# SonyCSLParis/audio-metrics

Measured on AMD Instinct MI355X. Metric: evaluate() embeddings/sec (FAD+KD+PRDC), 2×100k CLAP-512 sets, 1/2/4/8 GPUs, higher is better.
Workload: dtype f32

## Files before the change

audio-metrics_amd/csrc/am_common.h:

```cpp
#pragma once
#include <hip/hip_runtime.h>
#include <stdint.h>
#include <stddef.h>
#include <stdio.h>
#include "../../include/audio_metrics_hip.h"

namespace am {

char* last_error_buf();
void set_error(const char* fmt, ...);

#define AM_HIP_TRY(expr)                                                             \
    do {                                                                             \
        hipError_t _e = (expr);                                                      \
        if (_e != hipSuccess) {                                                      \
            am::set_error("%s failed: %s (%s:%d)", #expr, hipGetErrorString(_e),     \
                          __FILE__, __LINE__);                                       \
            return AM_ERR_HIP;                                                       \
        }                                                                            \
    } while (0)

#define AM_LAUNCH_CHECK()                                                            \
    do {                                                                             \
        hipError_t _e = hipGetLastError();                                           \
// ... 1 lines not shown
            am::set_error("kernel launch failed: %s (%s:%d)", hipGetErrorString(_e), \
                          __FILE__, __LINE__);                                       \
            return AM_ERR_HIP;                                                       \
        }                                                                            \
    } while (0)

#define AM_REQUIRE(cond, status, ...)                                                \
    do {                                                                             \
        if (!(cond)) {                                                               \
            am::set_error(__VA_ARGS__);                                              \
            return (status);                                                         \
        }                                                                            \
    } while (0)

hipError_t ensure_dynamic_lds(const void* kernel, int bytes);

void clock_begin(int kernel, hipStream_t st);
void clock_end(int kernel, hipStream_t st);

__device__ __forceinline__ float clamp0(float v) { return v != v ? __builtin_inff() : fmaxf(v, 0.f); }

static inline bool aligned16(const void* p) { return (reinterpret_cast<uintptr_t>(p) & 15u) == 0; }
static inline size_t round_up(size_t x, size_t a) { return (x + a - 1) / a * a; }
static inline int64_t ceil_div(int64_t a, int64_t b) { return (a + b - 1) / b; }

struct Carver {
    char* base;
    size_t size;
    size_t off = 0;
    Carver(void* p, size_t n) : base(static_cast<char*>(p)), size(n) {}
    template <class T>
    T* take(size_t count) {
        size_t bytes = round_up(count * sizeof(T), 256);
        T* r = (base && off + bytes <= size) ? reinterpret_cast<T*>(base + off) : nullptr;
        off += bytes;
        return r;
    }
    bool ok() const { return base != nullptr && off <= size; }
};

bool knn64_filter_eligible(int64_t N, int D, int k);
size_t knn64_filter_workspace(int64_t N, int D, int k);
int knn64_filter(const double* X, int64_t N, int64_t ld, int D, int k, double* out_r, void* ws, size_t ws_bytes, hipStream_t st);
bool prdc64_filter_eligible(int64_t Nr, int64_t Nc, int D);
size_t prdc64_filter_workspace(int64_t Nr, int64_t Nc, int D);
int prdc64_filter(const double* R, int64_t Nr, int64_t ldr, const double* C, int64_t Nc, int64_t ldc, int D, const double* rt,
                  const double* ct, int32_t* col_count, unsigned* row_any, unsigned* row_cover, const int** fail_flag, void* ws,
                  size_t ws_bytes, hipStream_t st);
size_t knn64_self_workspace(int64_t N, int k);
int knn64_self_gated(const double* X, int64_t N, int64_t ld, int D, int k, double* out_r, void* ws, size_t ws_bytes, const int* run_flag,
                     hipStream_t st);


}
```

audio-metrics_amd/csrc/evaluate.hip:

```cpp
#include "am_common.h"
#include <algorithm>
#include <vector>

namespace am {

__global__ void eval_pack_kernel(const double* __restrict__ fad5, const long long* __restrict__ totals, double* __restrict__ out,
                                 unsigned what) {
    const int t = threadIdx.x;
    if (t < AM_EVAL_HEAD) {
        double v = 0.0;
        if (t < 5) v = (what & AM_EVAL_FAD) ? fad5[t] : (t == 4 ? -1.0 : 0.0);
        else if (t < 9) v = (what & AM_EVAL_PRDC) ? (double)totals[t - 5] : 0.0;
        out[t] = v;
    }
}

struct EvalLayout {
    size_t total = 0;
    size_t stats_ws = 0, knn_ws = 0, prdc_ws = 0, kd_ws = 0, fad_ws = 0;
    double *mean[2] = {nullptr, nullptr}, *cov[2] = {nullptr, nullptr};
    float *norms[2] = {nullptr, nullptr}, *radii[2] = {nullptr, nullptr};
    uint32_t* pstats[2] = {nullptr, nullptr};
    uint16_t* half[2] = {nullptr, nullptr};
    int32_t* col = nullptr;
    uint8_t *rany = nullptr, *rcov = nullptr;
    long long* totals = nullptr;
    double* fad_out = nullptr;
    void *ws_main = nullptr, *ws_fad = nullptr;
    size_t ws_main_bytes = 0;
};

static bool eval_layout(Carver& c, int64_t n_ref, int64_t n_cand, int D, int k, int S, int m, unsigned what, EvalLayout& L) {
    const int64_t n[2] = {n_ref, n_cand};
    for (int s = 0; s < 2; ++s) {
        L.mean[s] = c.take<double>(D);
        L.cov[s] = c.take<double>((size_t)D * D);
    }
    size_t main_bytes = 0;
    if (what & AM_EVAL_FAD) {
        main_bytes = std::max({main_bytes, am_stats_workspace_bytes(n_ref, D), am_stats_workspace_bytes(n_cand, D)});
        L.fad_ws = am_frechet_workspace_bytes(D);
        L.ws_fad = c.take<char>(L.fad_ws);
        L.fad_out = c.take<double>(8);
    }
    if (what & AM_EVAL_PRDC) {
        const int64_t ldh = am_prepared_half_ld(D);
        for (int s = 0; s < 2; ++s) {
            L.norms[s] = c.take<float>(n[s]);
            L.pstats[s] = c.take<uint32_t>(4);
            L.half[s] = c.take<uint16_t>((size_t)n[s] * ldh);
            L.radii[s] = c.take<float>(n[s]);
        }
        L.col = c.take<int32_t>(n_cand);
        L.rany = c.take<uint8_t>(n_ref);
        L.rcov = c.take<uint8_t>(n_ref);
        L.totals = c.take<long long>(4);
        main_bytes = std::max({main_bytes, am_knn_workspace_bytes(n_ref, n_ref, D, k), am_knn_workspace_bytes(n_cand, n_cand, D, k),
                               am_prdc_workspace_bytes(n_ref, n_cand, D)});
    }
    if (what & AM_EVAL_KD) main_bytes = std::max(main_bytes, am_kd_poly_workspace_bytes(S, m, D));
    L.ws_main_bytes = round_up(std::max<size_t>(main_bytes, 256), 256);
    L.ws_main = c.take<char>(L.ws_main_bytes);
    L.total = c.off;
    return c.ok();
}

}

using namespace am;

extern "C" size_t am_evaluate_workspace_bytes(int64_t n_ref, int64_t n_cand, int D, int nearest_k, int kd_subsets, int kd_m,
                                              unsigned what) {
    if (n_ref < 1 || n_cand < 1 || D < 1) return 0;
    Carver c(nullptr, 0);
    EvalLayout L;
    eval_layout(c, n_ref, n_cand, D, nearest_k, kd_subsets, kd_m, what, L);
    return L.total;
}

extern "C" int am_evaluate_f32(const float* ref, int64_t n_ref, int64_t ld_ref, const float* cand, int64_t n_cand,
                               int64_t ld_cand, int D, unsigned what, int nearest_k, const int64_t* idx_cand,
                               const int64_t* idx_ref, int kd_subsets, int kd_m, double kd_gamma, double kd_coef0, int kd_degree,
                               const am_evaluate_side* given_ref, const am_evaluate_side* given_cand, double* out, void* ws,
                               size_t ws_bytes, am_stream_t stream, am_stream_t side_stream) {
    AM_REQUIRE(ref && cand && out, AM_ERR_BAD_ARG, "null pointer");
    AM_REQUIRE(n_ref >= 1 && n_cand >= 1 && D >= 1, AM_ERR_BAD_SHAPE, "sets of %lld and %lld rows x %d", (long long)n_ref,
               (long long)n_cand, D);
    AM_REQUIRE((what & ~(unsigned)(AM_EVAL_FAD | AM_EVAL_KD | AM_EVAL_PRDC)) == 0 && what != 0, AM_ERR_BAD_ARG, "what = %u", what);
    AM_REQUIRE(!(what & AM_EVAL_KD) || (idx_cand && idx_ref && kd_subsets >= 1 && kd_m >= 1), AM_ERR_BAD_ARG,
               "kernel distance needs the two index tables");
    AM_REQUIRE(!(what & AM_EVAL_FAD) || side_stream != stream, AM_ERR_BAD_ARG,
               "the Frechet solve runs on side_stream, which must differ from stream");
    hipStream_t st = static_cast<hipStream_t>(stream), side = static_cast<hipStream_t>(side_stream);
#ifdef AM_DEV_KNOBS
    static const int fad_place = getenv("AM_EVAL_FAD_PLACE") ? atoi(getenv("AM_EVAL_FAD_PLACE")) : 0;
#else
    constexpr int fad_place = 0;
#endif
    Carver c(ws, ws_bytes);
    EvalLayout L;
    AM_REQUIRE(eval_layout(c, n_ref, n_cand, D, nearest_k, kd_subsets, kd_m, what, L), AM_ERR_WORKSPACE,
               "workspace too small: need %zu bytes, have %zu", L.total, ws_bytes);
    const float* X[2] = {ref, cand};
    const int64_t n[2] = {n_ref, n_cand}, ld[2] = {ld_ref, ld_cand};
    const am_evaluate_side* given[2] = {given_ref, given_cand};
    int rc;

    const double* mean[2];
    const double* cov[2];
    if (what & AM_EVAL_FAD) {
        for (int s = 0; s < 2; ++s) {
            if (given[s] && given[s]->mean && given[s]->cov) {
                mean[s] = given[s]->mean;
                cov[s] = given[s]->cov;
                continue;
            }
            double* m_out = given[s] && given[s]->mean_out ? given[s]->mean_out : L.mean[s];
            double* c_out = given[s] && given[s]->cov_out ? given[s]->cov_out : L.cov[s];
            if ((rc = am_stats_f32(X[s], n[s], D, ld[s], m_out, c_out, L.ws_main, L.ws_main_bytes, stream)) != AM_OK) return rc;
            mean[s] = m_out;
            cov[s] = c_out;
        }
    }
    struct EventGuard {
        hipEvent_t e = nullptr;
        ~EventGuard() {
            if (e) (void)hipEventDestroy(e);
        }
    } ev_stats, ev_fad;
    if ((what & AM_EVAL_FAD) && fad_place != 2) {
        AM_HIP_TRY(hipEventCreateWithFlags(&ev_stats.e, hipEventDisableTiming));
        AM_HIP_TRY(hipEventRecord(ev_stats.e, st));
    }

    if (what & AM_EVAL_PRDC) {
        am_prepared_set prep[2];
        for (int s = 0; s < 2; ++s) {
            if ((rc = am_prepare_set_f32(X[s], n[s], ld[s], D, L.norms[s], L.pstats[s], L.half[s], stream)) != AM_OK) return rc;
            prep[s].norms = L.norms[s];
            prep[s].stats = L.pstats[s];
            prep[s].half = L.half[s];
        }
        const float* radii[2];
        for (int s = 0; s < 2; ++s) {
            if (given[s] && given[s]->radii) {
                radii[s] = given[s]->radii;
                continue;
            }
            float* r_out = given[s] && given[s]->radii_out ? given[s]->radii_out : L.radii[s];
            if ((rc = am_knn_radii_prepared_f32(X[s], n[s], ld[s], D, &prep[s], nearest_k, r_out, L.ws_main, L.ws_main_bytes,
                                                stream)) != AM_OK)
                return rc;
            radii[s] = r_out;
            if ((what & AM_EVAL_FAD) && fad_place == 2 && ev_stats.e == nullptr) {
                AM_HIP_TRY(hipEventCreateWithFlags(&ev_stats.e, hipEventDisableTiming));
                AM_HIP_TRY(hipEventRecord(ev_stats.e, st));
            }
        }
        if ((rc = am_prdc_counts_prepared_f32(ref, n_ref, ld_ref, &prep[0], cand, n_cand, ld_cand, &prep[1], D, radii[0], radii[1],
                                              L.col, L.rany, L.rcov, nullptr, L.ws_main, L.ws_main_bytes, stream)) != AM_OK)
            return rc;
        if ((rc = am_prdc_reduce(L.col, n_cand, L.rany, L.rcov, n_ref, reinterpret_cast<int64_t*>(L.totals), stream)) != AM_OK)
            return rc;
    }

    if (what & AM_EVAL_KD) {
        if ((rc = am_kd_poly_f32(cand, n_cand, ld_cand, ref, n_ref, ld_ref, D, idx_cand, idx_ref, kd_subsets, kd_m, kd_gamma,
                                 kd_coef0, kd_degree, out + AM_EVAL_HEAD, L.ws_main, L.ws_main_bytes, stream)) != AM_OK)
            return rc;
    }

    if (what & AM_EVAL_FAD) {
        const bool serial = fad_place == 1;
        if (!serial) {
            if (ev_stats.e == nullptr) {
                AM_HIP_TRY(hipEventCreateWithFlags(&ev_stats.e, hipEventDisableTiming));
                AM_HIP_TRY(hipEventRecord(ev_stats.e, st));
            }
            AM_HIP_TRY(hipStreamWaitEvent(side, ev_stats.e, 0));
        }
        const int block = am_frechet_first_block(), max_iter = 64;
        for (int first = 0; first < 2 * block; first += block)
            if ((rc = am_frechet_enqueue_f64(mean[1], cov[1], mean[0], cov[0], D, first, block, max_iter, 1e-13, L.fad_out,
                                             L.ws_fad, L.fad_ws, serial ? stream : side_stream)) != AM_OK)
                return rc;
        if (!serial) {
            AM_HIP_TRY(hipEventCreateWithFlags(&ev_fad.e, hipEventDisableTiming));
            AM_HIP_TRY(hipEventRecord(ev_fad.e, side));
            AM_HIP_TRY(hipStreamWaitEvent(st, ev_fad.e, 0));
        }
    }
// ... 358 lines not shown
```

audio-metrics_amd/csrc/pairwise.hip:

```cpp
#include "pairwise_common.h"
#include <algorithm>
#include <vector>
#include <cmath>
#include <type_traits>

namespace am {

__global__ void __launch_bounds__(256) row_sqnorm_kernel(const float* __restrict__ X, int64_t N, int64_t ld,
                                                         int D, float* __restrict__ out) {
    const int lane = threadIdx.x & 63;
    const int64_t row = (int64_t)blockIdx.x * 4 + (threadIdx.x >> 6);
    if (row >= N) return;
    const float* x = X + row * ld;
    float acc = 0.f;
    for (int k = lane * 4; k < D; k += 256) {
        const f32x4 v = load_k4(x, k, D);
        acc = fmaf(v.x, v.x, acc);
        acc = fmaf(v.y, v.y, acc);
        acc = fmaf(v.z, v.z, acc);
        acc = fmaf(v.w, v.w, acc);
    }
#pragma unroll
    for (int off = 32; off >= 1; off >>= 1) acc = acc + __shfl_xor(acc, off);
    if (lane == 0) out[row] = acc;
// ... 1259 lines not shown
    L.ld32 = (int64_t)round_up((size_t)D, (size_t)4);
    L.r32 = c.take<float>((size_t)Nr * L.ld32);
    L.c32 = c.take<float>((size_t)Nc * L.ld32);
    L.rn = c.take<float>(Nr);
    L.rt = c.take<float>(Nr);
    L.cn = c.take<float>(Nc);
    L.ct = c.take<float>(Nc);
    L.rmin = c.take<unsigned>(Nr);
    L.plan = plan_cross_fast(Nr, Nc, D);
    L.buf = carve_cross_fast(c, Nr, Nc, D, L.plan);
    L.total = c.off;
    return c.ok();
}
size_t prdc64_filter_workspace(int64_t Nr, int64_t Nc, int D) {
    Carver c(nullptr, 0);
    Prdc64Layout L;
    prdc64_layout(c, Nr, Nc, D, L);
    return L.total;
}

int prdc64_filter(const double* R, int64_t Nr, int64_t ldr, const double* C, int64_t Nc, int64_t ldc, int D, const double* rt,
                  const double* ct, int32_t* col_count, unsigned* row_any, unsigned* row_cover, const int** fail_flag, void* ws,
                  size_t ws_bytes, hipStream_t st) {
    Carver c(ws, ws_bytes);
    Prdc64Layout L;
    AM_REQUIRE(prdc64_layout(c, Nr, Nc, D, L), AM_ERR_WORKSPACE, "workspace too small: need %zu bytes, have %zu", L.total, ws_bytes);
    hipLaunchKernelGGL(cast64_kernel, dim3((unsigned)ceil_div(Nr * L.ld32, 256)), dim3(256), 0, st, R, Nr, ldr, D, L.r32, L.ld32);
    hipLaunchKernelGGL(cast64_kernel, dim3((unsigned)ceil_div(Nc * L.ld32, 256)), dim3(256), 0, st, C, Nc, ldc, D, L.c32, L.ld32);
    hipLaunchKernelGGL(narrow64_kernel, dim3((unsigned)ceil_div(Nr, 256)), dim3(256), 0, st, rt, Nr, L.rt);
    hipLaunchKernelGGL(narrow64_kernel, dim3((unsigned)ceil_div(Nc, 256)), dim3(256), 0, st, ct, Nc, L.ct);
    hipLaunchKernelGGL(fill_u32_kernel, dim3((unsigned)ceil_div(Nr, 256)), dim3(256), 0, st, L.rmin, Nr, 0x7f800000u);
    AM_LAUNCH_CHECK();
    int rc;
    if ((rc = norms_of(nullptr, L.r32, Nr, L.ld32, D, L.rn, st)) != AM_OK) return rc;
    if ((rc = norms_of(nullptr, L.c32, Nc, L.ld32, D, L.cn, st)) != AM_OK) return rc;
    const Prdc64Hook h{R, C, ldr, ldc, rt, ct};
    if ((rc = run_cross_fast(L.r32, Nr, L.ld32, L.rn, L.rt, L.c32, Nc, L.ld32, L.cn, L.ct, D, L.plan, L.buf, col_count, L.rmin, row_any,
                             row_cover, false, st, nullptr, nullptr, &h)) != AM_OK)
        return rc;
    *fail_flag = L.buf.ov_count + 1;
    return AM_OK;
}

}

extern "C" int am_knn_radii_f32(const float* X, int64_t N, int64_t ldx, const float* Y, int64_t M, int64_t ldy,
                                int D, int k, float* out_r, void* ws, size_t ws_bytes, am_stream_t stream) {
    return knn_radii_impl(X, N, ldx, Y, M, ldy, D, k, out_r, ws, ws_bytes, stream, nullptr);
}

static bool prepared_ok(const am_prepared_set* p) { return p != nullptr && p->norms != nullptr && p->stats != nullptr && p->half != nullptr; }
static PreparedSet prepared_of(const am_prepared_set* p) { return PreparedSet{p->norms, p->stats, p->half}; }

extern "C" int64_t am_prepared_half_ld(int D) { return D < 1 ? 0 : half_ld(D); }

extern "C" int am_prepare_set_f32(const float* X, int64_t N, int64_t ld, int D, float* norms, uint32_t* stats4, uint16_t* half,
                                  am_stream_t stream) {
    int rc;
    if ((rc = check_matrix(X, N, ld, D, "X")) != AM_OK) return rc;
    AM_REQUIRE(norms && stats4 && half, AM_ERR_BAD_ARG, "null output pointer");
    hipStream_t st = static_cast<hipStream_t>(stream);
    if ((rc = launch_norms(X, N, ld, D, norms, st)) != AM_OK) return rc;
    AM_HIP_TRY(hipMemsetAsync(stats4, 0, 4 * sizeof(unsigned), st));
    return launch_to_half(X, N, ld, D, norms, stats4, 0, half, st);
}

extern "C" int am_knn_radii_prepared_f32(const float* X, int64_t N, int64_t ldx, int D, const am_prepared_set* prepared, int k,
                                         float* out_r, void* ws, size_t ws_bytes, am_stream_t stream) {
    AM_REQUIRE(prepared_ok(prepared), AM_ERR_BAD_ARG, "prepared set has a null member");
    const PreparedSet ps = prepared_of(prepared);
    return knn_radii_impl(X, N, ldx, X, N, ldx, D, k, out_r, ws, ws_bytes, stream, &ps);
}

extern "C" int am_filter_stats_enable(int64_t* device_slots) {
    if (device_slots == nullptr) {
        g_filter_stats = nullptr;
        g_filter_stats_device = -1;
        return AM_OK;
    }
    int dev = -1;
    AM_HIP_TRY(hipGetDevice(&dev));
    g_filter_stats = reinterpret_cast<long long*>(device_slots);
    g_filter_stats_device = dev;
    return AM_OK;
}

extern "C" int am_knn_path(int64_t N, int64_t M, int D, int k, int self) {
    if (N < 1 || M < 1 || D < 1 || k < 1) return -1;
    if (k > AM_MAX_K) return 4;
    const KnnPlan p = plan_knn(N, M, D, k, self != 0 && N == M);
    return !p.sym ? 0 : (knn_fast_enabled(N, D) ? (p.tile_rows == 256 ? 3 : 2) : 1);
}
extern "C" int am_prdc_path(int64_t Nr, int64_t Nc, int D) {
    if (Nr < 1 || Nc < 1 || D < 1) return -1;
    if (!cross_fast_enabled(Nr, Nc, D)) return 0;
    return plan_cross_fast(Nr, Nc, D).wide ? 3 : 2;
}

extern "C" int am_filter_engine(int D) {
    if (D < 1) return 0;
    const int Dh = (int)(half_ld(D) / 2);
    return wide_stationary(Dh) ? (pstat64_supported(Dh) ? 2 : 1) : 0;
}

extern "C" int am_knn_sym_eligible(int64_t N, int D, int k) {
    if (N < 1 || D < 1 || k < 1 || k > AM_MAX_K) return 0;
// ... 324 lines not shown
```

audio-metrics_amd/csrc/stats.hip:

```cpp
#include "am_common.h"
#include "tile_engine.h"
#include <algorithm>

namespace am {

constexpr int SC_ROWS = 32;
constexpr int SC_LD = 128;
constexpr int SC_SLAB = SC_ROWS * SC_LD;
constexpr int SC_FLUSH = 8;

__global__ void __launch_bounds__(256) colsum_partial_kernel(const float* __restrict__ X, int64_t N, int64_t ld,
                                                             int D, int64_t rows_per_block,
                                                             double* __restrict__ partial) {
    __shared__ double red[256 * 4];
    const int tid = threadIdx.x;
    const int cgs = (D + 3) / 4;
    const int cpp = cgs < 256 ? cgs : 256;
    const int rpar = 256 / cpp;
    const int my_cg = tid % cpp, my_r = tid / cpp;
    const int64_t r0 = (int64_t)blockIdx.x * rows_per_block;
    const int64_t r1 = (r0 + rows_per_block < N) ? r0 + rows_per_block : N;
    for (int cg0 = 0; cg0 < cgs; cg0 += cpp) {
        const int cg = cg0 + my_cg;
        double s0 = 0, s1 = 0, s2 = 0, s3 = 0;
        if (cg < cgs && my_r < rpar) {
            int64_t row = r0 + my_r;
            for (; row + 3 * rpar < r1; row += 4 * rpar) {
                f32x4 v[4];
#pragma unroll
                for (int u = 0; u < 4; ++u) v[u] = load_k4(X + (row + u * rpar) * ld, cg * 4, D);
#pragma unroll
                for (int u = 0; u < 4; ++u) { s0 += (double)v[u].x; s1 += (double)v[u].y; s2 += (double)v[u].z; s3 += (double)v[u].w; }
            }
            for (; row < r1; row += rpar) {
                const f32x4 v = load_k4(X + row * ld, cg * 4, D);
                s0 += (double)v.x; s1 += (double)v.y; s2 += (double)v.z; s3 += (double)v.w;
            }
        }
        red[tid * 4 + 0] = s0; red[tid * 4 + 1] = s1; red[tid * 4 + 2] = s2; red[tid * 4 + 3] = s3;
        __syncthreads();
        if (my_r == 0 && cg < cgs) {
            for (int rr = 1; rr < rpar; ++rr) {
                const int o = (rr * cpp + my_cg) * 4;
                s0 += red[o]; s1 += red[o + 1]; s2 += red[o + 2]; s3 += red[o + 3];
            }
            double* out = partial + (int64_t)blockIdx.x * D + cg * 4;
            out[0] = s0;
            if (cg * 4 + 1 < D) out[1] = s1;
            if (cg * 4 + 2 < D) out[2] = s2;
            if (cg * 4 + 3 < D) out[3] = s3;
        }
        __syncthreads();
    }
}

constexpr int CSR_COLS = 16, CSR_PARTS = 16;
__global__ void __launch_bounds__(256) colsum_reduce_kernel(const double* __restrict__ partial, int nblocks, int D,
                                                            double scale, double* __restrict__ out) {
    __shared__ double red[CSR_PARTS][CSR_COLS];
    const int c = threadIdx.x % CSR_COLS, part = threadIdx.x / CSR_COLS;
    const int d = blockIdx.x * CSR_COLS + c;
    double s = 0;
    if (d < D) {
        int b = part;
        for (; b + 7 * CSR_PARTS < nblocks; b += 8 * CSR_PARTS) {
            double v[8];
#pragma unroll
            for (int u = 0; u < 8; ++u) v[u] = partial[(int64_t)(b + u * CSR_PARTS) * D + d];
#pragma unroll
            for (int u = 0; u < 8; ++u) s += v[u];
        }
        for (; b < nblocks; b += CSR_PARTS) s += partial[(int64_t)b * D + d];
    }
    red[part][c] = s;
    __syncthreads();
    if (part == 0 && d < D) {
        double t = red[0][c];
        for (int q = 1; q < CSR_PARTS; ++q) t += red[q][c];
        out[d] = t * scale;
    }
}

__device__ __forceinline__ void tri_decode(int t, int T, int& tp, int& tq) {
    tp = 0;
    int rem = t;
    while (rem >= T - tp) { rem -= T - tp; ++tp; }
    tq = tp + rem;
}

template <bool FULLD>
__global__ void __launch_bounds__(ENGINE_THREADS, 2)
scatter_partial_kernel(const float* __restrict__ X, int64_t N, int64_t ld, int D, const double* __restrict__ mean,
                       int64_t rows_per_slab, int ntri, double* __restrict__ partial) {
    __shared__ __attribute__((aligned(16))) float lds[4 * SC_SLAB];
    const LaneInfo L;
    const int T = (D + TB - 1) / TB;
    const int tri = blockIdx.x % ntri;
    const int slab = blockIdx.x / ntri;
    int tp, tq;
    tri_decode(tri, T, tp, tq);
    const int64_t r0 = (int64_t)slab * rows_per_slab;
    const int64_t r1 = (r0 + rows_per_slab < N) ? r0 + rows_per_slab : N;
    const int nstages = (int)((r1 - r0 + SC_ROWS - 1) / SC_ROWS);

    const int srow = L.tid >> 5, sc4 = (L.tid & 31) * 4;
    const int colA = tp * TB + sc4, colB = tq * TB + sc4;
    f32x4 muA, muB;
#pragma unroll
    for (int e = 0; e < 4; ++e) {
        muA[e] = (float)mean[colA + e < D ? colA + e : D - 1];
        muB[e] = (float)mean[colB + e < D ? colB + e : D - 1];
    }
    f32x4 ra[4], rb[4];
    const unsigned voA = (unsigned)((srow * ld + (colA + 3 < ld ? colA : 0)) * 4);
    const unsigned voB = (unsigned)((srow * ld + (colB + 3 < ld ? colB : 0)) * 4);
    const unsigned row_bytes = (unsigned)(ld * 4);
    auto issue = [&](int st) {
        const int64_t row0 = r0 + (int64_t)st * SC_ROWS;
        const int64_t left = r1 - row0;
        const float* p0 = X + row0 * ld;
        const unsigned lo = __builtin_amdgcn_readfirstlane((unsigned)(reinterpret_cast<uintptr_t>(p0) & 0xffffffffu));
        const unsigned hi = __builtin_amdgcn_readfirstlane((unsigned)(reinterpret_cast<uintptr_t>(p0) >> 32));
        const unsigned bytes = __builtin_amdgcn_readfirstlane((unsigned)((left < SC_ROWS ? left : SC_ROWS) * ld * 4));
        TileRsrc xr;
        xr.rsrc = __builtin_amdgcn_make_buffer_rsrc(reinterpret_cast<void*>((static_cast<uintptr_t>(hi) << 32) | lo), 0, (int)bytes, 0x00020000);
#pragma unroll
        for (int q = 0; q < 4; ++q) {
            ra[q] = rsrc_load(xr, voA, (unsigned)(q * 8) * row_bytes);
            rb[q] = rsrc_load(xr, voB, (unsigned)(q * 8) * row_bytes);
        }
    };
    const bool fullA = colA + 3 < D, fullB = colB + 3 < D;
    auto centre = [&](const f32x4& v, const f32x4& mu, int col, bool full, bool row_ok) {
// ... 52 lines not shown
#pragma unroll
            for (int a = 0; a < 2; ++a)
#pragma unroll
                for (int b = 0; b < 2; ++b)
#pragma unroll
                    for (int i = 0; i < 16; ++i) acc64[a][b][i] += (double)acc[a][b][i];
            zero_acc(acc);
        }
        if (more) commit(st + 1);
        __syncthreads();
    }
    double* out = partial + ((int64_t)slab * ntri + tri) * (TB * TB);
#pragma unroll
    for (int mt = 0; mt < 2; ++mt)
#pragma unroll
        for (int nt = 0; nt < 2; ++nt)
#pragma unroll
            for (int i = 0; i < 16; ++i) {
                const int p = L.wm * 64 + mt * 32 + (i & 3) + 8 * (i >> 2) + 4 * L.h;
                const int q = L.wn * 64 + nt * 32 + L.r;
                out[p * TB + q] = acc64[mt][nt][i];
            }
}

__global__ void __launch_bounds__(256) scatter_reduce_kernel(const double* __restrict__ partial, int nslabs, int ntri, int D, double scale,
                                                             double* __restrict__ out) {
    const int T = (D + TB - 1) / TB;
    const int tri = blockIdx.y;
    int tp, tq;
    tri_decode(tri, T, tp, tq);
    const int e = blockIdx.x * 256 + threadIdx.x;
    const int a = tp * TB + e / TB, b = tq * TB + e % TB;
    if (a >= D || b >= D) return;
    const double* src = partial + (int64_t)tri * (TB * TB) + e;
    const int64_t step = (int64_t)ntri * (TB * TB);
    double s = 0;
    int sl = 0;
    for (; sl + 7 < nslabs; sl += 8) {
        double v[8];
#pragma unroll
        for (int u = 0; u < 8; ++u) v[u] = src[(sl + u) * step];
#pragma unroll
        for (int u = 0; u < 8; ++u) s += v[u];
    }
    for (; sl < nslabs; ++sl) s += src[sl * step];
    s *= scale;
    out[(int64_t)a * D + b] = s;
    if (tp != tq) out[(int64_t)b * D + a] = s;
}

__global__ void zero_f64_kernel(double* __restrict__ p, int64_t n) {
    const int64_t i = (int64_t)blockIdx.x * blockDim.x + threadIdx.x;
    if (i < n) p[i] = 0.0;
}

__global__ void merge_cov_kernel(int64_t n1, const double* __restrict__ mean1, const double* cov1, int64_t n2,
                                 const double* __restrict__ mean2, const double* __restrict__ cov2, int D,
                                 double* out_cov) {
    const int j = blockIdx.x * blockDim.x + threadIdx.x;
    const int i = blockIdx.y;
    if (j >= D) return;
    const double n = (double)(n1 + n2);
    const double w1 = (double)(n1 - 1) / (n - 1);
    const double w2 = (double)(n2 - 1) / (n - 1);
    const double wd = ((double)n1 * (double)n2 / n) / (n - 1);
    const double di = mean1[i] - mean2[i], dj = mean1[j] - mean2[j];
    const int64_t o = (int64_t)i * D + j;
    out_cov[o] = (w1 * cov1[o] + w2 * cov2[o]) + wd * (di * dj);
}

__global__ void merge_mean_kernel(int64_t n1, const double* mean1, int64_t n2, const double* __restrict__ mean2, int D,
                                  double* out_mean) {
    const int i = blockIdx.x * blockDim.x + threadIdx.x;
    if (i >= D) return;
    out_mean[i] = ((double)n1 * mean1[i] + (double)n2 * mean2[i]) / (double)(n1 + n2);
}


constexpr int PUSH_TILE = 32;
constexpr int PUSH_MAX_ROWS = 128;

__global__ void __launch_bounds__(256) stats_push_kernel(const float* __restrict__ E, int b, int D, int64_t ld, int64_t n_old,
                                                         const double* __restrict__ mean_in, double* __restrict__ mean_out,
                                                         double* __restrict__ cov, float* __restrict__ rows_out, int64_t ld_out) {
    __shared__ float ea[PUSH_MAX_ROWS][PUSH_TILE + 1], eb[PUSH_MAX_ROWS][PUSH_TILE + 1];
    __shared__ double mu[2][PUSH_TILE];
    const int tid = threadIdx.x;
    const int tj = blockIdx.x, ti = blockIdx.y;
    const int i0 = ti * PUSH_TILE, j0 = tj * PUSH_TILE;
    for (int e = tid; e < b * PUSH_TILE; e += 256) {
        const int r = e / PUSH_TILE, c = e % PUSH_TILE;
        ea[r][c] = i0 + c < D ? E[(int64_t)r * ld + i0 + c] : 0.f;
        eb[r][c] = j0 + c < D ? E[(int64_t)r * ld + j0 + c] : 0.f;
    }
    __syncthreads();
    if (tid < 2 * PUSH_TILE) {
        const int which = tid / PUSH_TILE, c = tid % PUSH_TILE;
        double s = 0;
        for (int r = 0; r < b; ++r) s += (double)(which ? eb[r][c] : ea[r][c]);
        mu[which][c] = s / (double)b;
    }
    __syncthreads();
    for (int e = tid; e < b * PUSH_TILE; e += 256) {
        const int r = e / PUSH_TILE, c = e % PUSH_TILE;
        ea[r][c] -= (float)mu[0][c];
        eb[r][c] -= (float)mu[1][c];
// ... 134 lines not shown
    if (tp != tq || j > i) out[(int64_t)j * D + i] = s;
}

struct Stats64Plan {
    int cs_blocks, ntri, nslabs;
    int64_t cs_rows, slab_rows;
};
static Stats64Plan plan_stats64(int64_t N, int D) {
    Stats64Plan p;
    int64_t b = std::min<int64_t>(std::max<int64_t>(ceil_div(N, 256), 1), 512);
    p.cs_rows = ceil_div(N, b);
    p.cs_blocks = (int)ceil_div(N, p.cs_rows);
    const int T = (int)ceil_div(D, S64_TILE);
    p.ntri = T * (T + 1) / 2;
    int64_t s = std::max<int64_t>(2048 / p.ntri, 1);
    s = std::min<int64_t>(s, std::max<int64_t>(ceil_div(N, 256), 1));
    s = std::min<int64_t>(s, 64);
    p.slab_rows = ceil_div(ceil_div(N, s), 16) * 16;
    p.nslabs = (int)ceil_div(N, p.slab_rows);
    return p;
}
static size_t stats64_ws(int D, const Stats64Plan& p) {
    Carver c(nullptr, 0);
    c.take<double>((size_t)p.cs_blocks * D);
    c.take<double>((size_t)p.nslabs * p.ntri * S64_TILE * S64_TILE);
    return c.off;
}

static int run_colsum(const float* X, int64_t N, int D, int64_t ld, double scale, double* out, double* partial,
                      const StatsPlan& p, hipStream_t st) {
    hipLaunchKernelGGL(colsum_partial_kernel, dim3(p.cs_blocks), dim3(256), 0, st, X, N, ld, D, p.cs_rows, partial);
    AM_LAUNCH_CHECK();
    hipLaunchKernelGGL(colsum_reduce_kernel, dim3((unsigned)ceil_div(D, CSR_COLS)), dim3(256), 0, st, partial, p.cs_blocks, D,
                       scale, out);
    AM_LAUNCH_CHECK();
    return AM_OK;
}

static int run_scatter(const float* X, int64_t N, int D, int64_t ld, const double* mean, double scale, double* out,
                       double* partial, const StatsPlan& p, hipStream_t st) {
    if (D % TB == 0)
        hipLaunchKernelGGL(scatter_partial_kernel<true>, dim3((unsigned)(p.ntri * p.nslabs)), dim3(ENGINE_THREADS), 0, st, X, N, ld,
                           D, mean, p.slab_rows, p.ntri, partial);
    else
        hipLaunchKernelGGL(scatter_partial_kernel<false>, dim3((unsigned)(p.ntri * p.nslabs)), dim3(ENGINE_THREADS), 0, st, X, N, ld,
                           D, mean, p.slab_rows, p.ntri, partial);
    AM_LAUNCH_CHECK();
    hipLaunchKernelGGL(scatter_reduce_kernel, dim3((unsigned)(TB * TB / 256), (unsigned)p.ntri), dim3(256), 0, st, partial,
                       p.nslabs, p.ntri, D, scale, out);
    AM_LAUNCH_CHECK();
    return AM_OK;
}

}

using namespace am;

extern "C" size_t am_stats_workspace_bytes(int64_t N, int D) {
    if (N < 1 || D < 1) return 0;
    return stats_ws(N, D, plan_stats(N, D));
}

extern "C" int am_colsum_f32(const float* X, int64_t N, int D, int64_t ld, double* colsum, void* ws, size_t ws_bytes,
                             am_stream_t stream) {
    int rc;
    if ((rc = check_x(X, N, D, ld)) != AM_OK) return rc;
    AM_REQUIRE(colsum != nullptr, AM_ERR_BAD_ARG, "colsum is null");
    const StatsPlan p = plan_stats(N, D);
    Carver c(ws, ws_bytes);
    double* cs_part = c.take<double>((size_t)p.cs_blocks * D);
    AM_REQUIRE(c.ok(), AM_ERR_WORKSPACE, "workspace too small: need %zu bytes, have %zu", c.off, ws_bytes);
    return run_colsum(X, N, D, ld, 1.0, colsum, cs_part, p, static_cast<hipStream_t>(stream));
}

extern "C" int am_scatter_f32(const float* X, int64_t N, int D, int64_t ld, const double* mean, double* scatter,
                              void* ws, size_t ws_bytes, am_stream_t stream) {
    int rc;
    if ((rc = check_x(X, N, D, ld)) != AM_OK) return rc;
    AM_REQUIRE(mean && scatter, AM_ERR_BAD_ARG, "mean/scatter is null");
    const StatsPlan p = plan_stats(N, D);
    Carver c(ws, ws_bytes);
    c.take<double>((size_t)p.cs_blocks * D);
    double* sc_part = c.take<double>((size_t)p.nslabs * p.ntri * TB * TB);
    AM_REQUIRE(c.ok(), AM_ERR_WORKSPACE, "workspace too small: need %zu bytes, have %zu", c.off, ws_bytes);
    return run_scatter(X, N, D, ld, mean, 1.0, scatter, sc_part, p, static_cast<hipStream_t>(stream));
}

extern "C" int am_stats_f32(const float* X, int64_t N, int D, int64_t ld, double* mean, double* cov, void* ws,
                            size_t ws_bytes, am_stream_t stream) {
    int rc;
    if ((rc = check_x(X, N, D, ld)) != AM_OK) return rc;
    AM_REQUIRE(mean && cov, AM_ERR_BAD_ARG, "mean/cov is null");
    hipStream_t st = static_cast<hipStream_t>(stream);
    const StatsPlan p = plan_stats(N, D);
    Carver c(ws, ws_bytes);
    double* cs_part = c.take<double>((size_t)p.cs_blocks * D);
    double* sc_part = c.take<double>((size_t)p.nslabs * p.ntri * TB * TB);
    AM_REQUIRE(c.ok(), AM_ERR_WORKSPACE, "workspace too small: need %zu bytes, have %zu", c.off, ws_bytes);
    if ((rc = run_colsum(X, N, D, ld, 1.0 / (double)N, mean, cs_part, p, st)) != AM_OK) return rc;
    if (N == 1) {
        hipLaunchKernelGGL(zero_f64_kernel, dim3((unsigned)ceil_div((int64_t)D * D, 256)), dim3(256), 0, st, cov,
                           (int64_t)D * D);
        AM_LAUNCH_CHECK();
        return AM_OK;
    }
    return run_scatter(X, N, D, ld, mean, 1.0 / (double)(N - 1), cov, sc_part, p, st);
}

extern "C" size_t am_stats_f64_workspace_bytes(int64_t N, int D) {
    if (N < 1 || D < 1) return 0;
    return stats64_ws(D, plan_stats64(N, D));
}

static int check_x64(const double* X, int64_t N, int D, int64_t ld) {
    AM_REQUIRE(X != nullptr, AM_ERR_BAD_ARG, "X is null");
    AM_REQUIRE(N >= 1 && D >= 1, AM_ERR_BAD_SHAPE, "X has shape %lld x %d", (long long)N, D);
    AM_REQUIRE(D <= 8192, AM_ERR_BAD_SHAPE, "float64 statistics take rows of up to 8192 elements (D=%d)", D);
    AM_REQUIRE(ld >= D, AM_ERR_BAD_ARG, "ld=%lld < D=%d", (long long)ld, D);
    return AM_OK;
}

static int run_colsum64(const double* X, int64_t N, int D, int64_t ld, double scale, double* out, double* cs_part, const Stats64Plan& p,
                        hipStream_t st) {
    hipLaunchKernelGGL(colsum64_partial_kernel, dim3(p.cs_blocks), dim3(256), 0, st, X, N, ld, D, p.cs_rows, cs_part);
    AM_LAUNCH_CHECK();
    hipLaunchKernelGGL(colsum_reduce_kernel, dim3((unsigned)ceil_div(D, CSR_COLS)), dim3(256), 0, st, cs_part, p.cs_blocks, D, scale, out);
    AM_LAUNCH_CHECK();
    return AM_OK;
}

static int run_scatter64(const double* X, int64_t N, int D, int64_t ld, const double* mean, double scale, double* out, double* sc_part,
                         const Stats64Plan& p, hipStream_t st) {
    hipLaunchKernelGGL(scatter64_partial_kernel, dim3((unsigned)(p.ntri * p.nslabs)), dim3(256), 0, st, X, N, ld, D, mean, p.slab_rows,
                       p.ntri, sc_part);
    AM_LAUNCH_CHECK();
    hipLaunchKernelGGL(scatter64_reduce_kernel, dim3(S64_TILE * S64_TILE / 256, (unsigned)p.ntri), dim3(256), 0, st, sc_part,
                       p.nslabs, p.ntri, D, scale, out);
    AM_LAUNCH_CHECK();
    return AM_OK;
}

extern "C" int am_colsum_f64(const double* X, int64_t N, int D, int64_t ld, double* colsum, void* ws, size_t ws_bytes, am_stream_t stream) {
    int rc;
    if ((rc = check_x64(X, N, D, ld)) != AM_OK) return rc;
    AM_REQUIRE(colsum != nullptr, AM_ERR_BAD_ARG, "colsum is null");
    const Stats64Plan p = plan_stats64(N, D);
// ... 71 lines not shown
```

Baseline: 8.501 million.

## Fuse FAD stats with PRDC set preparation into shared scan and split-f16 scatter

Adds a scan kernel that computes column sums, row norms and max statistics in one pass, and a scatter kernel that uses split-f16 MFMA (hi/lo products) to build the covariance. On the diagonal tiles it also writes the scaled half-precision copy that PRDC needs. In evaluate(), when both FAD and PRDC are requested, this replaces the separate am_stats_f32 and am_prepare_set_f32 passes, aiming to cut repeated reads of the input and the FP64 scatter cost. The standalone stats entry points are also routed through the new path. The split-f16 scatter trades some covariance accuracy for speed and adds a larger workspace requirement.

```diff
diff --git a/audio-metrics_amd/csrc/am_common.h b/audio-metrics_amd/csrc/am_common.h
--- a/audio-metrics_amd/csrc/am_common.h
+++ b/audio-metrics_amd/csrc/am_common.h
@@ -77,4 +77,11 @@
                      hipStream_t st);
 
 
+bool fused_prepare_eligible(int64_t N, int D);
+size_t fused_prepare_workspace_bytes(int64_t N, int D);
+int fused_prepare_stats_f32(const float* X, int64_t N, int64_t ld, int D, double* mean, double* cov, float* norms, unsigned* stats4,
+                            uint16_t* half, int64_t ldh, int drop, void* ws, size_t ws_bytes, hipStream_t st);
+int prepared_half_drop_bits();
+
+
 }
diff --git a/audio-metrics_amd/csrc/evaluate.hip b/audio-metrics_amd/csrc/evaluate.hip
--- a/audio-metrics_amd/csrc/evaluate.hip
+++ b/audio-metrics_amd/csrc/evaluate.hip
@@ -57,6 +57,9 @@
         L.totals = c.take<long long>(4);
         main_bytes = std::max({main_bytes, am_knn_workspace_bytes(n_ref, n_ref, D, k), am_knn_workspace_bytes(n_cand, n_cand, D, k),
                                am_prdc_workspace_bytes(n_ref, n_cand, D)});
+        if (what & AM_EVAL_FAD)
+            for (int s = 0; s < 2; ++s)
+                if (fused_prepare_eligible(n[s], D)) main_bytes = std::max(main_bytes, fused_prepare_workspace_bytes(n[s], D));
     }
     if (what & AM_EVAL_KD) main_bytes = std::max(main_bytes, am_kd_poly_workspace_bytes(S, m, D));
     L.ws_main_bytes = round_up(std::max<size_t>(main_bytes, 256), 256);
@@ -108,6 +111,7 @@
 
     const double* mean[2];
     const double* cov[2];
+    bool prepared[2] = {false, false};
     if (what & AM_EVAL_FAD) {
         for (int s = 0; s < 2; ++s) {
             if (given[s] && given[s]->mean && given[s]->cov) {
@@ -117,7 +121,14 @@
             }
             double* m_out = given[s] && given[s]->mean_out ? given[s]->mean_out : L.mean[s];
             double* c_out = given[s] && given[s]->cov_out ? given[s]->cov_out : L.cov[s];
-            if ((rc = am_stats_f32(X[s], n[s], D, ld[s], m_out, c_out, L.ws_main, L.ws_main_bytes, stream)) != AM_OK) return rc;
+            if ((what & AM_EVAL_PRDC) && fused_prepare_eligible(n[s], D)) {
+                if ((rc = fused_prepare_stats_f32(X[s], n[s], ld[s], D, m_out, c_out, L.norms[s], L.pstats[s], L.half[s], am_prepared_half_ld(D),
+                                                  prepared_half_drop_bits(), L.ws_main, L.ws_main_bytes, st)) != AM_OK)
+                    return rc;
+                prepared[s] = true;
+            } else if ((rc = am_stats_f32(X[s], n[s], D, ld[s], m_out, c_out, L.ws_main, L.ws_main_bytes, stream)) != AM_OK) {
+                return rc;
+            }
             mean[s] = m_out;
             cov[s] = c_out;
         }
@@ -136,7 +147,8 @@
     if (what & AM_EVAL_PRDC) {
         am_prepared_set prep[2];
         for (int s = 0; s < 2; ++s) {
-            if ((rc = am_prepare_set_f32(X[s], n[s], ld[s], D, L.norms[s], L.pstats[s], L.half[s], stream)) != AM_OK) return rc;
+            if (!prepared[s] && (rc = am_prepare_set_f32(X[s], n[s], ld[s], D, L.norms[s], L.pstats[s], L.half[s], stream)) != AM_OK)
+                return rc;
             prep[s].norms = L.norms[s];
             prep[s].stats = L.pstats[s];
             prep[s].half = L.half[s];
diff --git a/audio-metrics_amd/csrc/pairwise.hip b/audio-metrics_amd/csrc/pairwise.hip
--- a/audio-metrics_amd/csrc/pairwise.hip
+++ b/audio-metrics_amd/csrc/pairwise.hip
@@ -1335,6 +1335,10 @@
 static bool prepared_ok(const am_prepared_set* p) { return p != nullptr && p->norms != nullptr && p->stats != nullptr && p->half != nullptr; }
 static PreparedSet prepared_of(const am_prepared_set* p) { return PreparedSet{p->norms, p->stats, p->half}; }
 
+namespace am {
+int prepared_half_drop_bits() { return half_drop_bits(); }
+}
+
 extern "C" int64_t am_prepared_half_ld(int D) { return D < 1 ? 0 : half_ld(D); }
 
 extern "C" int am_prepare_set_f32(const float* X, int64_t N, int64_t ld, int D, float* norms, uint32_t* stats4, uint16_t* half,
diff --git a/audio-metrics_amd/csrc/stats.hip b/audio-metrics_amd/csrc/stats.hip
--- a/audio-metrics_amd/csrc/stats.hip
+++ b/audio-metrics_amd/csrc/stats.hip
@@ -1,5 +1,6 @@
 #include "am_common.h"
 #include "tile_engine.h"
+#include "pairwise_common.h"
 #include <algorithm>
 
 namespace am {
@@ -55,8 +56,8 @@
 }
 
 constexpr int CSR_COLS = 16, CSR_PARTS = 16;
-__global__ void __launch_bounds__(256) colsum_reduce_kernel(const double* __restrict__ partial, int nblocks, int D,
-                                                            double scale, double* __restrict__ out) {
+__device__ __forceinline__ void colsum_reduce_block(const double* __restrict__ partial, int nblocks, int D, double scale,
+                                                    double* __restrict__ out) {
     __shared__ double red[CSR_PARTS][CSR_COLS];
     const int c = threadIdx.x % CSR_COLS, part = threadIdx.x / CSR_COLS;
     const int d = blockIdx.x * CSR_COLS + c;
@@ -79,6 +80,11 @@
         for (int q = 1; q < CSR_PARTS; ++q) t += red[q][c];
         out[d] = t * scale;
     }
+}
+
+__global__ void __launch_bounds__(256) colsum_reduce_kernel(const double* __restrict__ partial, int nblocks, int D,
+                                                            double scale, double* __restrict__ out) {
+    colsum_reduce_block(partial, nblocks, D, scale, out);
 }
 
 __device__ __forceinline__ void tri_decode(int t, int T, int& tp, int& tq) {
@@ -237,6 +243,273 @@
 __global__ void zero_f64_kernel(double* __restrict__ p, int64_t n) {
     const int64_t i = (int64_t)blockIdx.x * blockDim.x + threadIdx.x;
     if (i < n) p[i] = 0.0;
+}
+
+
+template <int NC>
+__global__ void __launch_bounds__(256) prep_scan_kernel(const float* __restrict__ X, int64_t N, int64_t ld, int D,
+                                                        int64_t rows_per_block, float* __restrict__ norms,
+                                                        double* __restrict__ col_part, unsigned* __restrict__ max_part) {
+    __shared__ double red[4][NC * 256];
+    __shared__ unsigned mred[4][2];
+    const int lane = threadIdx.x & 63, wave = threadIdx.x >> 6;
+    const int64_t r0 = (int64_t)blockIdx.x * rows_per_block;
+    const int64_t r1 = (r0 + rows_per_block < N) ? r0 + rows_per_block : N;
+    double cs[NC][4];
+#pragma unroll
+    for (int c = 0; c < NC; ++c)
+#pragma unroll
+        for (int e = 0; e < 4; ++e) cs[c][e] = 0.0;
+    unsigned mabs = 0u, mnorm = 0u;
+    for (int64_t row = r0 + wave * 4; row < r1; row += 16) {
+        f32x4 v[4][NC];
+#pragma unroll
+        for (int u = 0; u < 4; ++u)
+#pragma unroll
+            for (int c = 0; c < NC; ++c) v[u][c] = load_k4(row + u < r1 ? X + (row + u) * ld : nullptr, lane * 4 + 256 * c, D);
+#pragma unroll
+        for (int u = 0; u < 4; ++u) {
+            float acc = 0.f;
+#pragma unroll
+            for (int c = 0; c < NC; ++c) {
+                const f32x4 x = v[u][c];
+                if (lane * 4 + 256 * c < D) {
+                    acc = fmaf(x.x, x.x, acc);
+                    acc = fmaf(x.y, x.y, acc);
+                    acc = fmaf(x.z, x.z, acc);
+                    acc = fmaf(x.w, x.w, acc);
+                }
+                cs[c][0] += (double)x.x; cs[c][1] += (double)x.y; cs[c][2] += (double)x.z; cs[c][3] += (double)x.w;
+                mabs = max(max(mabs, __float_as_uint(x.x) & 0x7fffffffu), __float_as_uint(x.y) & 0x7fffffffu);
+                mabs = max(max(mabs, __float_as_uint(x.z) & 0x7fffffffu), __float_as_uint(x.w) & 0x7fffffffu);
+            }
+#pragma unroll
+            for (int off = 32; off >= 1; off >>= 1) acc = acc + __shfl_xor(acc, off);
+            if (row + u < r1) {
+                if (lane == 0) norms[row + u] = acc;
+                mnorm = max(mnorm, __float_as_uint(acc));
+            }
+        }
+    }
+#pragma unroll
+    for (int c = 0; c < NC; ++c)
+#pragma unroll
+        for (int e = 0; e < 4; ++e) red[wave][256 * c + 4 * lane + e] = cs[c][e];
+#pragma unroll
+    for (int off = 32; off >= 1; off >>= 1) mabs = max(mabs, (unsigned)__shfl_xor((int)mabs, off));
+    if (lane == 0) {
+        mred[wave][0] = mnorm;
+        mred[wave][1] = mabs;
+    }
+    __syncthreads();
+    for (int d = threadIdx.x; d < D; d += 256)
+        col_part[(int64_t)blockIdx.x * D + d] = ((red[0][d] + red[1][d]) + red[2][d]) + red[3][d];
+    if (threadIdx.x < 2)
+        max_part[2 * blockIdx.x + threadIdx.x] =
+            max(max(mred[0][threadIdx.x], mred[1][threadIdx.x]), max(mred[2][threadIdx.x], mred[3][threadIdx.x]));
+}
+
+__global__ void __launch_bounds__(256) prep_scan_reduce_kernel(const double* __restrict__ partial, const unsigned* __restrict__ max_part,
+                                                               int nblocks, int D, double scale, double* __restrict__ mean,
+                                                               unsigned* __restrict__ stats4) {
+    colsum_reduce_block(partial, nblocks, D, scale, mean);
+    if (blockIdx.x != 0) return;
+    unsigned a = 0u, b = 0u;
+    for (int i = threadIdx.x; i < nblocks; i += 256) {
+        a = max(a, max_part[2 * i]);
+        b = max(b, max_part[2 * i + 1]);
+    }
+#pragma unroll
+    for (int off = 32; off >= 1; off >>= 1) {
+        a = max(a, (unsigned)__shfl_xor((int)a, off));
+        b = max(b, (unsigned)__shfl_xor((int)b, off));
+    }
+    __shared__ unsigned m[4][2];
+    if ((threadIdx.x & 63) == 0) {
+        m[threadIdx.x >> 6][0] = a;
+        m[threadIdx.x >> 6][1] = b;
+    }
+    __syncthreads();
+    if (threadIdx.x < 4) {
+        const int w = threadIdx.x >> 1;
+        stats4[threadIdx.x] = (threadIdx.x & 1) ? 0u : max(max(m[0][w], m[1][w]), max(m[2][w], m[3][w]));
+    }
+}
+
+constexpr int SP_ROWS = 32;
+constexpr int SP_IMG = TB * SP_ROWS;
+constexpr int SP_FLUSH = 8;
+typedef _Float16 f16x4s __attribute__((ext_vector_type(4)));
+
+__device__ __forceinline__ int sp_off(int col, int chunk) { return col * SP_ROWS + ((chunk ^ ((col >> 2) & 3)) << 3); }
+
+template <bool FULLD>
+__global__ void __launch_bounds__(ENGINE_THREADS, 1)
+scatter_split_kernel(const float* __restrict__ X, int64_t N, int64_t ld, int D, const double* __restrict__ mean,
+                     const unsigned* __restrict__ stats4, int64_t rows_per_slab, int ntri, double* __restrict__ partial,
+                     uint16_t* __restrict__ Xh, int64_t ldh, int drop) {
+    __shared__ __attribute__((aligned(16))) _Float16 lds[2][4][SP_IMG];
+    const LaneInfo L;
+    const int T = (D + TB - 1) / TB;
+    const int tri = blockIdx.x % ntri;
+    const int slab = blockIdx.x / ntri;
+    int tp, tq;
+    tri_decode(tri, T, tp, tq);
+    const bool diag = tp == tq;
+    const int64_t r0 = (int64_t)slab * rows_per_slab;
+    const int64_t r1 = (r0 + rows_per_slab < N) ? r0 + rows_per_slab : N;
+    const int nstages = (int)((r1 - r0 + SP_ROWS - 1) / SP_ROWS);
+
+    const int rg = L.tid & 7, cg = L.tid >> 3;
+    const int colA = tp * TB + 4 * cg, colB = tq * TB + 4 * cg;
+    f32x4 muA, muB;
+#pragma unroll
+    for (int e = 0; e < 4; ++e) {
+        muA[e] = (float)mean[colA + e < D ? colA + e : D - 1];
+        muB[e] = (float)mean[colB + e < D ? colB + e : D - 1];
+    }
+    const unsigned mb = stats4[2];
+    const int ex = 13 - ((mb == 0u || mb >= 0x7f800000u) ? 13 : (int)((mb >> 23) & 255u) - 127);
+    const float sa = ldexpf(1.f, ex / 2), sb = ldexpf(1.f, ex - ex / 2);
+    const float hsc = __uint_as_float((unsigned)(127 + half_scale_exp(mb)) << 23);
+
+    f32x4 ra[4], rb[4];
+    const unsigned voA = (unsigned)((4 * rg * ld + (colA + 3 < ld ? colA : 0)) * 4);
+    const unsigned voB = (unsigned)((4 * rg * ld + (colB + 3 < ld ? colB : 0)) * 4);
+    const unsigned row_bytes = (unsigned)(ld * 4);
+    auto issue = [&](int st) {
+        const int64_t row0 = r0 + (int64_t)st * SP_ROWS;
+        const int64_t left = r1 - row0;
+        const float* p0 = X + row0 * ld;
+        const unsigned lo = __builtin_amdgcn_readfirstlane((unsigned)(reinterpret_cast<uintptr_t>(p0) & 0xffffffffu));
+        const unsigned hi = __builtin_amdgcn_readfirstlane((unsigned)(reinterpret_cast<uintptr_t>(p0) >> 32));
+        const unsigned bytes = __builtin_amdgcn_readfirstlane((unsigned)((left < SP_ROWS ? left : SP_ROWS) * ld * 4));
+        TileRsrc xr;
+        xr.rsrc = __builtin_amdgcn_make_buffer_rsrc(reinterpret_cast<void*>((static_cast<uintptr_t>(hi) << 32) | lo), 0, (int)bytes, 0x00020000);
+#pragma unroll
+        for (int q = 0; q < 4; ++q) ra[q] = rsrc_load(xr, voA, (unsigned)q * row_bytes);
+        if (!diag) {
+#pragma unroll
+            for (int q = 0; q < 4; ++q) rb[q] = rsrc_load(xr, voB, (unsigned)q * row_bytes);
+        }
+    };
+    const bool fullA = colA + 3 < D, fullB = colB + 3 < D;
+    auto stage_op = [&](const f32x4 (&v)[4], const f32x4& mu, int col, bool full, bool whole, int64_t row0, _Float16* img) {
+        f32x4 xs[4];
+#pragma unroll
+        for (int q = 0; q < 4; ++q) {
+            const bool row_ok = whole || row0 + 4 * rg + q < r1;
+#pragma unroll
+            for (int e = 0; e < 4; ++e) {
+                const bool ok = (FULLD && whole) || (row_ok && (full || col + e < D));
+                xs[q][e] = ok ? ((v[q][e] - mu[e]) * sa) * sb : 0.f;
+            }
+        }
+#pragma unroll
+        for (int e = 0; e < 4; ++e) {
+            f16x4s h, l;
+#pragma unroll
+            for (int q = 0; q < 4; ++q) {
+                h[q] = (_Float16)xs[q][e];
+                l[q] = (_Float16)(xs[q][e] - (float)h[q]);
+            }
+            const int o = sp_off(4 * cg + e, rg >> 1) + (rg & 1) * 4;
+            *reinterpret_cast<f16x4s*>(img + o) = h;
+            *reinterpret_cast<f16x4s*>(img + SP_IMG + o) = l;
+        }
+    };
+    auto half_copy = [&](int64_t row0, bool whole) {
+        if (colA >= ldh) return;
+#pragma unroll
+        for (int q = 0; q < 4; ++q) {
+            const int64_t row = row0 + 4 * rg + q;
+            if (!whole && row >= r1) continue;
+            unsigned b[4];
+#pragma unroll
+            for (int e = 0; e < 4; ++e) {
+                const float v = (FULLD || colA + e < D) ? ra[q][e] : 0.f;
+                unsigned u = (unsigned)__builtin_bit_cast(unsigned short, (_Float16)(v * hsc));
+                if (drop > 0) {
+                    const unsigned mag = u & 0x7fffu;
+                    u = (u & 0x8000u) | ((mag + (1u << (drop - 1)) - 1u + ((mag >> drop) & 1u)) & ~((1u << drop) - 1u));
+                }
+                b[e] = u;
+            }
+            uint2 o;
+            o.x = b[0] | (b[1] << 16);
+            o.y = b[2] | (b[3] << 16);
+            *reinterpret_cast<uint2*>(Xh + row * ldh + colA) = o;
+        }
+    };
+    auto commit = [&](int st) {
+        _Float16* img = &lds[st & 1][0][0];
+        const int64_t row0 = r0 + (int64_t)st * SP_ROWS;
+        const bool whole = row0 + SP_ROWS <= r1;
+        stage_op(ra, muA, colA, fullA, whole, row0, img);
+        if (!diag) stage_op(rb, muB, colB, fullB, whole, row0, img + 2 * SP_IMG);
+        else if (Xh != nullptr) half_copy(row0, whole);
+    };
+
+    f32x16 acc[2][2];
+    zero_acc(acc);
+    double acc64[2][2][16];
+#pragma unroll
+    for (int a = 0; a < 2; ++a)
+#pragma unroll
+        for (int b = 0; b < 2; ++b)
+#pragma unroll
+            for (int i = 0; i < 16; ++i) acc64[a][b][i] = 0.0;
+
+    if (nstages > 0) {
+        issue(0);
+        commit(0);
+    }
+    __syncthreads();
+    for (int st = 0; st < nstages; ++st) {
+        const bool more = st + 1 < nstages;
+        if (more) issue(st + 1);
+        const _Float16* sA = &lds[st & 1][0][0];
+        const _Float16* sB = diag ? sA : sA + 2 * SP_IMG;
+#pragma unroll
+        for (int ks = 0; ks < SP_ROWS / 16; ++ks) {
+#pragma unroll
+            for (int mt = 0; mt < 2; ++mt) {
+                const int oa = sp_off(L.wm * 64 + mt * 32 + L.r, 2 * ks + L.h);
+                const f16x8 ah = *reinterpret_cast<const f16x8*>(sA + oa), al = *reinterpret_cast<const f16x8*>(sA + SP_IMG + oa);
+#pragma unroll
+                for (int nt = 0; nt < 2; ++nt) {
+                    const int ob = sp_off(L.wn * 64 + nt * 32 + L.r, 2 * ks + L.h);
+                    const f16x8 bh = *reinterpret_cast<const f16x8*>(sB + ob), bl = *reinterpret_cast<const f16x8*>(sB + SP_IMG + ob);
+                    acc[mt][nt] = __builtin_amdgcn_mfma_f32_32x32x16_f16(ah, bh, acc[mt][nt], 0, 0, 0);
+                    acc[mt][nt] = __builtin_amdgcn_mfma_f32_32x32x16_f16(ah, bl, acc[mt][nt], 0, 0, 0);
+                    acc[mt][nt] = __builtin_amdgcn_mfma_f32_32x32x16_f16(al, bh, acc[mt][nt], 0, 0, 0);
+                }
+            }
+        }
+        if ((st % SP_FLUSH) == SP_FLUSH - 1 || !more) {
+#pragma unroll
+            for (int a = 0; a < 2; ++a)
+#pragma unroll
+                for (int b = 0; b < 2; ++b)
+#pragma unroll
+                    for (int i = 0; i < 16; ++i) acc64[a][b][i] += (double)acc[a][b][i];
+            zero_acc(acc);
+        }
+        if (more) commit(st + 1);
+        __syncthreads();
+    }
+    const double unscale = ldexp(1.0, -2 * ex);
+    double* out = partial + ((int64_t)slab * ntri + tri) * (TB * TB);
+#pragma unroll
+    for (int mt = 0; mt < 2; ++mt)
+#pragma unroll
+        for (int nt = 0; nt < 2; ++nt)
+#pragma unroll
+            for (int i = 0; i < 16; ++i) {
+                const int p = L.wm * 64 + mt * 32 + (i & 3) + 8 * (i >> 2) + 4 * L.h;
+                const int q = L.wn * 64 + nt * 32 + L.r;
+                out[p * TB + q] = acc64[mt][nt][i] * unscale;
+            }
 }
 
 __global__ void merge_cov_kernel(int64_t n1, const double* __restrict__ mean1, const double* cov1, int64_t n2,
@@ -477,13 +750,119 @@
     return AM_OK;
 }
 
+constexpr int64_t FUSED_MIN_ROWS = 8192;
+constexpr int FUSED_MIN_DIM = 128, FUSED_MAX_DIM = 1024;
+
+struct FusedPlan {
+    int scan_blocks;
+    int64_t scan_rows;
+    StatsPlan sc;
+};
+static FusedPlan plan_fused(int64_t N, int D) {
+    FusedPlan p;
+    const int64_t b = std::min<int64_t>(std::max<int64_t>(ceil_div(N, 32), 1), 1024);
+    p.scan_rows = ceil_div(N, b);
+    p.scan_blocks = (int)ceil_div(N, p.scan_rows);
+    p.sc = plan_stats(N, D);
+    return p;
+}
+
+bool fused_prepare_eligible(int64_t N, int D) { return N >= FUSED_MIN_ROWS && D >= FUSED_MIN_DIM && D <= FUSED_MAX_DIM; }
+
+size_t fused_prepare_workspace_bytes(int64_t N, int D) {
+    const FusedPlan p = plan_fused(N, D);
+    Carver c(nullptr, 0);
+    c.take<double>((size_t)p.scan_blocks * D);
+    c.take<unsigned>((size_t)2 * p.scan_blocks);
+    c.take<double>((size_t)p.sc.nslabs * p.sc.ntri * TB * TB);
+    return c.off;
+}
+
+static int fused_scan(const float* X, int64_t N, int64_t ld, int D, double mean_scale, double* colsum, float* norms, unsigned* stats4,
+                      void* ws, size_t ws_bytes, hipStream_t st) {
+    const FusedPlan p = plan_fused(N, D);
+    Carver c(ws, ws_bytes);
+    double* col_part = c.take<double>((size_t)p.scan_blocks * D);
+    unsigned* max_part = c.take<unsigned>((size_t)2 * p.scan_blocks);
+    AM_REQUIRE(c.ok(), AM_ERR_WORKSPACE, "workspace too small: need %zu bytes, have %zu", c.off, ws_bytes);
+    if (D <= 256)
+        hipLaunchKernelGGL(prep_scan_kernel<1>, dim3(p.scan_blocks), dim3(256), 0, st, X, N, ld, D, p.scan_rows, norms, col_part, max_part);
+    else if (D <= 512)
+        hipLaunchKernelGGL(prep_scan_kernel<2>, dim3(p.scan_blocks), dim3(256), 0, st, X, N, ld, D, p.scan_rows, norms, col_part, max_part);
+    else
+        hipLaunchKernelGGL(prep_scan_kernel<4>, dim3(p.scan_blocks), dim3(256), 0, st, X, N, ld, D, p.scan_rows, norms, col_part, max_part);
+    AM_LAUNCH_CHECK();
+    hipLaunchKernelGGL(prep_scan_reduce_kernel, dim3((unsigned)ceil_div(D, CSR_COLS)), dim3(256), 0, st, col_part, max_part, p.scan_blocks,
+                       D, mean_scale, colsum, stats4);
+    AM_LAUNCH_CHECK();
+    return AM_OK;
+}
+
+static int fused_split(const float* X, int64_t N, int64_t ld, int D, const double* mean, const unsigned* stats4, double cov_scale,
+                       double* cov, uint16_t* half, int64_t ldh, int drop, void* ws, size_t ws_bytes, hipStream_t st) {
+    const FusedPlan p = plan_fused(N, D);
+    Carver c(ws, ws_bytes);
+    c.take<double>((size_t)p.scan_blocks * D);
+    c.take<unsigned>((size_t)2 * p.scan_blocks);
+    double* sc_part = c.take<double>((size_t)p.sc.nslabs * p.sc.ntri * TB * TB);
+    AM_REQUIRE(c.ok(), AM_ERR_WORKSPACE, "workspace too small: need %zu bytes, have %zu", c.off, ws_bytes);
+    const unsigned grid = (unsigned)(p.sc.ntri * p.sc.nslabs);
+    if (D % TB == 0)
+        hipLaunchKernelGGL(scatter_split_kernel<true>, dim3(grid), dim3(ENGINE_THREADS), 0, st, X, N, ld, D, mean, stats4, p.sc.slab_rows,
+                           p.sc.ntri, sc_part, half, ldh, drop);
+    else
+        hipLaunchKernelGGL(scatter_split_kernel<false>, dim3(grid), dim3(ENGINE_THREADS), 0, st, X, N, ld, D, mean, stats4, p.sc.slab_rows,
+                           p.sc.ntri, sc_part, half, ldh, drop);
+    AM_LAUNCH_CHECK();
+    hipLaunchKernelGGL(scatter_reduce_kernel, dim3((unsigned)(TB * TB / 256), (unsigned)p.sc.ntri), dim3(256), 0, st, sc_part,
+                       p.sc.nslabs, p.sc.ntri, D, cov_scale, cov);
+    AM_LAUNCH_CHECK();
+    return AM_OK;
+}
+
+int fused_prepare_stats_f32(const float* X, int64_t N, int64_t ld, int D, double* mean, double* cov, float* norms, unsigned* stats4,
+                            uint16_t* half, int64_t ldh, int drop, void* ws, size_t ws_bytes, hipStream_t st) {
+    int rc;
+    if ((rc = check_x(X, N, D, ld)) != AM_OK) return rc;
+    AM_REQUIRE(fused_prepare_eligible(N, D), AM_ERR_BAD_SHAPE, "fused prepare of %lld x %d", (long long)N, D);
+    if ((rc = fused_scan(X, N, ld, D, 1.0 / (double)N, mean, norms, stats4, ws, ws_bytes, st)) != AM_OK) return rc;
+    return fused_split(X, N, ld, D, mean, stats4, 1.0 / (double)(N - 1), cov, half, ldh, drop, ws, ws_bytes, st);
+}
+
 }
 
 using namespace am;
+
+static size_t stats_fused_ws(int64_t N, int D) {
+    Carver c(nullptr, 0);
+    c.take<char>(fused_prepare_workspace_bytes(N, D));
+    c.take<float>(N);
+    c.take<unsigned>(4);
+    c.take<double>(D);
+    return c.off;
+}
+
+struct FusedScratch {
+    void* ws;
+    size_t bytes;
+    float* norms;
+    unsigned* stats4;
+    double* colsum;
+};
+static bool fused_scratch(int64_t N, int D, void* ws, size_t ws_bytes, FusedScratch& f) {
+    Carver c(ws, ws_bytes);
+    f.bytes = fused_prepare_workspace_bytes(N, D);
+    f.ws = c.take<char>(f.bytes);
+    f.norms = c.take<float>(N);
+    f.stats4 = c.take<unsigned>(4);
+    f.colsum = c.take<double>(D);
+    return c.ok();
+}
 
 extern "C" size_t am_stats_workspace_bytes(int64_t N, int D) {
     if (N < 1 || D < 1) return 0;
-    return stats_ws(N, D, plan_stats(N, D));
+    const size_t b = stats_ws(N, D, plan_stats(N, D));
+    return fused_prepare_eligible(N, D) ? std::max(b, stats_fused_ws(N, D)) : b;
 }
 
 extern "C" int am_colsum_f32(const float* X, int64_t N, int D, int64_t ld, double* colsum, void* ws, size_t ws_bytes,
@@ -491,6 +870,12 @@
     int rc;
     if ((rc = check_x(X, N, D, ld)) != AM_OK) return rc;
     AM_REQUIRE(colsum != nullptr, AM_ERR_BAD_ARG, "colsum is null");
+    if (fused_prepare_eligible(N, D)) {
+        FusedScratch f;
+        AM_REQUIRE(fused_scratch(N, D, ws, ws_bytes, f), AM_ERR_WORKSPACE, "workspace too small: need %zu bytes, have %zu",
+                   stats_fused_ws(N, D), ws_bytes);
+        return fused_scan(X, N, ld, D, 1.0, colsum, f.norms, f.stats4, f.ws, f.bytes, static_cast<hipStream_t>(stream));
+    }
     const StatsPlan p = plan_stats(N, D);
     Carver c(ws, ws_bytes);
     double* cs_part = c.take<double>((size_t)p.cs_blocks * D);
@@ -503,6 +888,14 @@
     int rc;
     if ((rc = check_x(X, N, D, ld)) != AM_OK) return rc;
     AM_REQUIRE(mean && scatter, AM_ERR_BAD_ARG, "mean/scatter is null");
+    if (fused_prepare_eligible(N, D)) {
+        hipStream_t st = static_cast<hipStream_t>(stream);
+        FusedScratch f;
+        AM_REQUIRE(fused_scratch(N, D, ws, ws_bytes, f), AM_ERR_WORKSPACE, "workspace too small: need %zu bytes, have %zu",
+                   stats_fused_ws(N, D), ws_bytes);
+        if ((rc = fused_scan(X, N, ld, D, 1.0, f.colsum, f.norms, f.stats4, f.ws, f.bytes, st)) != AM_OK) return rc;
+        return fused_split(X, N, ld, D, mean, f.stats4, 1.0, scatter, nullptr, 0, 0, f.ws, f.bytes, st);
+    }
     const StatsPlan p = plan_stats(N, D);
     Carver c(ws, ws_bytes);
     c.take<double>((size_t)p.cs_blocks * D);
@@ -517,6 +910,12 @@
     if ((rc = check_x(X, N, D, ld)) != AM_OK) return rc;
     AM_REQUIRE(mean && cov, AM_ERR_BAD_ARG, "mean/cov is null");
     hipStream_t st = static_cast<hipStream_t>(stream);
+    if (fused_prepare_eligible(N, D)) {
+        FusedScratch f;
+        AM_REQUIRE(fused_scratch(N, D, ws, ws_bytes, f), AM_ERR_WORKSPACE, "workspace too small: need %zu bytes, have %zu",
+                   stats_fused_ws(N, D), ws_bytes);
+        return fused_prepare_stats_f32(X, N, ld, D, mean, cov, f.norms, f.stats4, nullptr, 0, 0, f.ws, f.bytes, st);
+    }
     const StatsPlan p = plan_stats(N, D);
     Carver c(ws, ws_bytes);
     double* cs_part = c.take<double>((size_t)p.cs_blocks * D);
```

After: 8.618 million, median of 6. About the same (+1.4%).
